# kzhai/PyLDA

Hardware: AMD Instinct MI355X
Metric: documents/sec per VB iteration (higher is better)
Workload: dtype f64

## Files before the change

include/pylda_hip.h:

```cpp
#ifndef PYLDA_HIP_H
#define PYLDA_HIP_H

#include <stdint.h>

#ifdef __cplusplus
extern "C" {
#endif

typedef struct pylda_ctx pylda_ctx;
typedef struct pylda_corpus pylda_corpus;

typedef enum pylda_status {
    PYLDA_OK = 0,
    PYLDA_ERR_INVALID = -1,
    PYLDA_ERR_HIP = -2,
    PYLDA_ERR_OOM = -3,
    PYLDA_ERR_STATE = -4
} pylda_status;

#define PYLDA_ABI_VERSION 10
int pylda_abi_version(void);

const char* pylda_version(void);

// ... 77 lines not shown
int pylda_work_counters(pylda_ctx* ctx, double* inner_iterations, double* inner_iteration_terms);
int pylda_executed_work(pylda_ctx* ctx, double* tile_entries, double* handed_over);
int pylda_stop_sum_counters(pylda_ctx* ctx, double* skipped, double* formed);
int pylda_clock_counters(pylda_ctx* ctx, double* shader_ticks, double* wall_ticks, double* wall_hz);

int pylda_corpus_plan(pylda_corpus* corpus, int32_t capacity, int32_t* variant, int32_t* geometry,
                      int64_t* documents, int64_t* terms, double* kernel_ms);

int64_t pylda_corpus_layout(pylda_corpus* corpus, const char* name);

int pylda_set_option(pylda_ctx* ctx, const char* name, int64_t value);

int pylda_test_special(pylda_ctx* ctx, int64_t n, const double* x, double* digamma_out,
                       double* lgamma_out);

int pylda_parse_corpus(const char* text, int64_t text_bytes, int doc_separator, const char* vocab,
                       int64_t vocab_bytes, int lowercase, int64_t* n_docs, int64_t* nnz,
                       int64_t* doc_ptr, int32_t* term_id, int32_t* term_ct, int64_t* dropped_docs);

int pylda_test_alpha_update(pylda_ctx* ctx, const double* alpha_k, const double* alpha_ss_k, double number_of_documents,
                            int hyper_parameter_iteration, double hyper_parameter_decay_factor,
                            int hyper_parameter_maximum_decay, double hyper_parameter_converge_threshold,
                            double* alpha_out_k);

int pylda_hybrid_estep(pylda_ctx* ctx, pylda_corpus* corpus, int number_of_samples, int burn_in_samples, uint64_t seed,
                       uint64_t stream, int64_t first_document, int heldout);
int pylda_hybrid_scale_sstats(pylda_ctx* ctx, double divisor);

int pylda_test_philox(pylda_ctx* ctx, int64_t n, const uint32_t* counter_key, uint32_t* out);

int pylda_gibbs_init(pylda_ctx* ctx, pylda_corpus* corpus, uint64_t seed, int64_t first_document);
int pylda_gibbs_sweep(pylda_ctx* ctx, pylda_corpus* corpus, const double* alpha_k, const double* beta_v, double beta_sum,
                      int64_t blocks, uint64_t seed, uint64_t stream, int64_t first_document);
int pylda_gibbs_log_posterior(pylda_ctx* ctx, pylda_corpus* corpus, const double* alpha_k, const double* beta_v, double* out);
int pylda_gibbs_get_counts(pylda_ctx* ctx, pylda_corpus* corpus, int32_t* n_kv, int32_t* n_k, int32_t* topics);
int pylda_gibbs_set_state(pylda_ctx* ctx, pylda_corpus* corpus, const int32_t* n_kv, const int32_t* n_k, const int32_t* topics);

int pylda_gibbs_round_tokens(pylda_ctx* ctx, pylda_corpus* corpus, int64_t blocks, int64_t first_document, int64_t* tokens);
int pylda_gibbs_exchange_prepare(pylda_ctx* ctx, pylda_corpus* corpus, int64_t blocks, int64_t first_document, int world, int rank,
                                 const int64_t* capacity, void** send, void** recv);
int pylda_gibbs_round_sample(pylda_ctx* ctx, pylda_corpus* corpus, const double* alpha_k, const double* beta_v, double beta_sum,
                             int64_t blocks, int64_t round, uint64_t seed, uint64_t stream, int64_t first_document);
int pylda_gibbs_round_apply(pylda_ctx* ctx, pylda_corpus* corpus, int64_t round);
int pylda_gibbs_table_device(pylda_ctx* ctx, pylda_corpus* corpus, void** table, int64_t* table_elements, void** n_k);
int pylda_gibbs_log_posterior_parts(pylda_ctx* ctx, pylda_corpus* corpus, const double* alpha_k, const double* beta_v, double* out);

// ... 59 lines not shown
```

pylda_amd/_capi.py:

```python
import collections
import ctypes
import os
import threading

import numpy as np

ABI_VERSION = 10
_LIB_PATH = os.path.join(os.path.dirname(os.path.abspath(__file__)), "lib", "libpylda_hip.so")
_lib = None

_c_double_p = ctypes.POINTER(ctypes.c_double)
_c_int32_p = ctypes.POINTER(ctypes.c_int32)
_c_int64_p = ctypes.POINTER(ctypes.c_int64)
_vp = ctypes.c_void_p

SIGNATURES = {
    "pylda_version": (ctypes.c_char_p, []),
    "pylda_abi_version": (ctypes.c_int, []),
    "pylda_device_count": (ctypes.c_int, [ctypes.POINTER(ctypes.c_int)]),
    "pylda_create": (ctypes.c_int, [ctypes.c_int, ctypes.c_int, ctypes.c_int, ctypes.POINTER(_vp)]),
    "pylda_destroy": (None, [_vp]),
    "pylda_last_error": (ctypes.c_char_p, [_vp]),
    "pylda_set_stream": (ctypes.c_int, [_vp, _vp]),
    "pylda_use_own_stream": (ctypes.c_int, [_vp]),
# ... 38 lines not shown
    "pylda_host_free": (ctypes.c_int, [_vp]),
    "pylda_model_checkpoint": (ctypes.c_int, [_vp, ctypes.c_int]),
    "pylda_mark_time": (ctypes.c_int, [_vp, ctypes.c_int]),
    "pylda_elapsed_ms": (ctypes.c_int, [_vp, ctypes.c_int, ctypes.c_int, _c_double_p]),
    "pylda_work_counters": (ctypes.c_int, [_vp, _c_double_p, _c_double_p]),
    "pylda_executed_work": (ctypes.c_int, [_vp, _c_double_p, _c_double_p]),
    "pylda_stop_sum_counters": (ctypes.c_int, [_vp, _c_double_p, _c_double_p]),
    "pylda_clock_counters": (ctypes.c_int, [_vp, _c_double_p, _c_double_p, _c_double_p]),
    "pylda_set_profiling": (ctypes.c_int, [_vp, ctypes.c_int]),
    "pylda_kernel_time": (ctypes.c_int, [_vp, _c_double_p, _c_double_p, _c_int64_p]),
    "pylda_corpus_layout": (ctypes.c_int64, [_vp, ctypes.c_char_p]),
    "pylda_corpus_plan": (ctypes.c_int, [_vp, ctypes.c_int32, _c_int32_p, _c_int32_p, _c_int64_p, _c_int64_p,
                                         _c_double_p]),
    "pylda_set_option": (ctypes.c_int, [_vp, ctypes.c_char_p, ctypes.c_int64]),
    "pylda_parse_corpus": (ctypes.c_int, [ctypes.c_char_p, ctypes.c_int64, ctypes.c_int, ctypes.c_char_p,
                                          ctypes.c_int64, ctypes.c_int, _c_int64_p, _c_int64_p, _c_int64_p,
                                          _c_int32_p, _c_int32_p, _c_int64_p]),
    "pylda_test_alpha_update": (ctypes.c_int, [_vp, _c_double_p, _c_double_p, ctypes.c_double, ctypes.c_int, ctypes.c_double,
                                               ctypes.c_int, ctypes.c_double, _c_double_p]),
    "pylda_test_expdigamma": (ctypes.c_int, [_vp, ctypes.c_int64, _c_double_p, ctypes.c_double, _c_double_p]),
    "pylda_test_special_forms": (ctypes.c_int, [_vp, ctypes.c_int64, _c_double_p, ctypes.c_double, ctypes.c_int, _c_double_p]),
    "pylda_test_tables": (ctypes.c_int, [_vp, _c_double_p, _c_double_p, _c_double_p, _c_double_p, _c_double_p, _c_double_p,
                                         _c_double_p, ctypes.POINTER(ctypes.c_int)]),
    "pylda_test_statistics": (ctypes.c_int, [_vp, _vp, _c_double_p, _c_double_p, _c_int32_p, ctypes.POINTER(ctypes.c_uint16),
                                             _c_double_p, _c_double_p]),
    "pylda_test_special": (ctypes.c_int, [_vp, ctypes.c_int64, _c_double_p, _c_double_p, _c_double_p]),
    "pylda_test_gibbs_posterior_terms": (ctypes.c_int, [_vp, _vp, _c_double_p, _c_double_p, _c_double_p, _c_double_p, _c_double_p]),
    "pylda_hybrid_estep": (ctypes.c_int, [_vp, _vp, ctypes.c_int, ctypes.c_int, ctypes.c_uint64, ctypes.c_uint64,
                                          ctypes.c_int64, ctypes.c_int]),
    "pylda_hybrid_scale_sstats": (ctypes.c_int, [_vp, ctypes.c_double]),
    "pylda_test_philox": (ctypes.c_int, [_vp, ctypes.c_int64, ctypes.POINTER(ctypes.c_uint32),
                                         ctypes.POINTER(ctypes.c_uint32)]),
    "pylda_gibbs_init": (ctypes.c_int, [_vp, _vp, ctypes.c_uint64, ctypes.c_int64]),
    "pylda_gibbs_sweep": (ctypes.c_int, [_vp, _vp, _c_double_p, _c_double_p, ctypes.c_double, ctypes.c_int64, ctypes.c_uint64,
                                         ctypes.c_uint64, ctypes.c_int64]),
    "pylda_gibbs_log_posterior": (ctypes.c_int, [_vp, _vp, _c_double_p, _c_double_p, _c_double_p]),
    "pylda_gibbs_get_counts": (ctypes.c_int, [_vp, _vp, _c_int32_p, _c_int32_p, _c_int32_p]),
    "pylda_gibbs_set_state": (ctypes.c_int, [_vp, _vp, _c_int32_p, _c_int32_p, _c_int32_p]),
    "pylda_gibbs_round_tokens": (ctypes.c_int, [_vp, _vp, ctypes.c_int64, ctypes.c_int64, _c_int64_p]),
    "pylda_gibbs_exchange_prepare": (ctypes.c_int, [_vp, _vp, ctypes.c_int64, ctypes.c_int64, ctypes.c_int, ctypes.c_int, _c_int64_p,
                                                    ctypes.POINTER(_vp), ctypes.POINTER(_vp)]),
    "pylda_gibbs_round_sample": (ctypes.c_int, [_vp, _vp, _c_double_p, _c_double_p, ctypes.c_double, ctypes.c_int64, ctypes.c_int64,
                                                ctypes.c_uint64, ctypes.c_uint64, ctypes.c_int64]),
    "pylda_gibbs_round_apply": (ctypes.c_int, [_vp, _vp, ctypes.c_int64]),
    "pylda_gibbs_table_device": (ctypes.c_int, [_vp, _vp, ctypes.POINTER(_vp), _c_int64_p, ctypes.POINTER(_vp)]),
    "pylda_gibbs_log_posterior_parts": (ctypes.c_int, [_vp, _vp, _c_double_p, _c_double_p, _c_double_p]),
# ... 624 lines not shown

    def allreduce_doubles(self, values):
        values = np.ascontiguousarray(values, dtype=np.float64).copy()
        self._check(self._lib.pylda_allreduce_doubles(self._h, _dp(values), values.size))
        return values

    def set_profiling(self, enabled):
        self._check(self._lib.pylda_set_profiling(self._h, 1 if enabled else 0))

    def kernel_time(self):
        ms, ss, calls = ctypes.c_double(0), ctypes.c_double(0), ctypes.c_int64(0)
        self._check(self._lib.pylda_kernel_time(self._h, ctypes.byref(ms), ctypes.byref(ss), ctypes.byref(calls)))
        return ms.value, ss.value, calls.value

    def test_alpha_update(self, alpha, alpha_ss, number_of_documents, iterations=100, decay_factor=0.9, maximum_decay=10,
                          threshold=1e-6):
        alpha, alpha_ss = _f64(alpha, (self.K,), "alpha"), _f64(alpha_ss, (self.K,), "alpha_ss")
        out = np.empty(self.K, dtype=np.float64)
        self._check(self._lib.pylda_test_alpha_update(self._h, _dp(alpha), _dp(alpha_ss), float(number_of_documents),
                                                      int(iterations), float(decay_factor), int(maximum_decay),
                                                      float(threshold), _dp(out)))
        return out

    def test_expdigamma(self, x, c):
        x = _f64(x)
        out = np.empty_like(x)
        self._check(self._lib.pylda_test_expdigamma(self._h, x.size, _dp(x), float(c), _dp(out)))
        return out

    def test_special_forms(self, x, form, c=0.0):
        x = _f64(x)
        out = np.empty_like(x)
        self._check(self._lib.pylda_test_special_forms(self._h, x.size, _dp(x), float(c), int(form), _dp(out)))
        return out

    def test_special(self, x):
        x = _f64(x)
        dg, lg = np.empty_like(x), np.empty_like(x)
        self._check(self._lib.pylda_test_special(self._h, x.size, _dp(x), _dp(dg), _dp(lg)))
        return dg, lg

    def test_tables(self, alpha_sgn=False, tables=True, only=None):
        ldk = int(self._lib.pylda_table_stride(self._h))
        out = {}
        if tables:
            out = {"psi_rowsum": (self.K,), "elog": (self.V, ldk), "expElog": (self.V, ldk),
# ... 117 lines not shown
```

pylda_amd/csrc/context.hip:

```cpp
#include "host_internal.h"
#include "transpose_kernel.h"
#include "special_device.h"

namespace pylda_host {

std::string g_create_error;

int fail(pylda_ctx* ctx, int code, const char* fmt, ...)
{
    char buf[512];
    va_list ap;
    va_start(ap, fmt);
    vsnprintf(buf, sizeof buf, fmt, ap);
    va_end(ap);
    if (ctx) ctx->err = buf; else g_create_error = buf;
    return code;
}

static hipEvent_t take_event(pylda_ctx* ctx)
{
    if (!ctx->event_pool.empty()) {
        hipEvent_t e = ctx->event_pool.back();
        ctx->event_pool.pop_back();
        return e;
// ... 138 lines not shown
    for (int i = 0; i < pylda_ctx::kAux; ++i) {
        CREATE_TRY(hip_ok(hipStreamCreateWithFlags(&ctx->aux_stream[i], hipStreamNonBlocking), "hipStreamCreate"));
        CREATE_TRY(hip_ok(hipEventCreateWithFlags(&ctx->join_event[i], hipEventDisableTiming), "hipEventCreate"));
    }
    CREATE_TRY(hip_ok(hipEventCreateWithFlags(&ctx->fork_event, hipEventDisableTiming), "hipEventCreate"));
    const size_t kv = (size_t)K * V, wk = (size_t)V * ctx->ldk;
    CREATE_TRY(dev_alloc(ctx, &ctx->d_eta, kv));
    CREATE_TRY(dev_alloc(ctx, &ctx->d_elog, wk));
    CREATE_TRY(dev_alloc(ctx, &ctx->d_expElog, wk));
    CREATE_TRY(dev_alloc(ctx, &ctx->d_expElog_elog, wk));
    CREATE_TRY(dev_alloc(ctx, &ctx->d_sstats, wk));
    CREATE_TRY(dev_alloc(ctx, &ctx->d_kv_scratch, kv));
    CREATE_TRY(dev_alloc(ctx, &ctx->d_shift, (size_t)V));
    CREATE_TRY(dev_alloc(ctx, &ctx->d_beta, (size_t)V));
    CREATE_TRY(dev_alloc(ctx, &ctx->d_psi_rowsum, (size_t)K));
    CREATE_TRY(dev_alloc(ctx, &ctx->d_topic_lse, (size_t)K));
    CREATE_TRY(dev_alloc(ctx, &ctx->d_alpha, (size_t)K));
    CREATE_TRY(dev_alloc(ctx, &ctx->d_alpha_sgn, (size_t)K));
    CREATE_TRY(dev_alloc(ctx, &ctx->d_alpha_wsum, (size_t)1));
    CREATE_TRY(dev_alloc(ctx, &ctx->d_small, (size_t)(4 * K + 16)));
    CREATE_TRY(dev_alloc(ctx, &ctx->d_partial, (size_t)1024 * K));
    CREATE_TRY(dev_alloc(ctx, &ctx->d_outer, (size_t)(3 * K + 8)));
    CREATE_TRY(dev_alloc(ctx, &ctx->d_newton_work, (size_t)4 * K));
    CREATE_TRY(dev_alloc(ctx, &ctx->d_work, (size_t)8));
    CREATE_TRY(hip_ok(hipMemsetAsync(ctx->d_work, 0, 8 * sizeof(double), ctx->stream), "hipMemsetAsync"));
    CREATE_TRY(hip_ok(hipHostMalloc(reinterpret_cast<void**>(&ctx->h_pin), (size_t)(5 * K + 8) * sizeof(double), hipHostMallocDefault),
                      "hipHostMalloc"));
    for (int i = 0; i < 2; ++i)
        CREATE_TRY(hip_ok(hipEventCreateWithFlags(&ctx->alpha_event[i], hipEventDisableTiming), "hipEventCreate"));
    CREATE_TRY(hip_ok(hipMemsetAsync(ctx->d_sstats, 0, wk * sizeof(double), ctx->stream),
                      "hipMemsetAsync"));
#undef CREATE_TRY
    *out = ctx;
    return PYLDA_OK;
}

void pylda_destroy(pylda_ctx* ctx)
{
    if (!ctx) return;
    (void)hipSetDevice(ctx->device);
    if (ctx->own_stream) (void)hipStreamSynchronize(ctx->own_stream);
    if (ctx->comm) pylda::comm_destroy(ctx->comm);
    dev_free(ctx->d_comm_small);
    dev_free(ctx->d_foldin_table); dev_free(ctx->d_foldin_alpha); dev_free(ctx->d_completion_rowsum);
    dev_free(ctx->d_similarity_base);
    dev_free(ctx->d_ltr_z); dev_free(ctx->d_ltr_p);
    drain_events(ctx);
// ... 79 lines not shown
        ctx->wide_postings = value != 0;
    } else if (!strcmp(name, "lds_pad")) {
        ctx->lds_pad = (int)value;
    } else if (!strcmp(name, "quad")) {
        ctx->quad = value != 0;
        ctx->plan_epoch += 1;
    } else if (!strcmp(name, "quad_stream")) {
        ctx->quad_stream = value != 0;
        ctx->plan_epoch += 1;
    } else if (!strcmp(name, "quad_packed")) {
        ctx->quad_packed = value != 0;
    } else if (!strcmp(name, "prepare_path")) {
        if (value < 0 || value > 2 || (value == 1 && ctx->K > 64))
            return fail(ctx, PYLDA_ERR_INVALID, "prepare_path=%lld at K=%d: 0 (by size), 1 (one kernel, K <= 64) or 2 (two passes)",
                        (long long)value, ctx->K);
        ctx->prepare_path = (int)value;
    } else if (!strcmp(name, "quilt12")) {
        ctx->quilt12 = value != 0;
        ctx->plan_epoch += 1;
    } else if (!strcmp(name, "doc_values")) {
        ctx->doc_values = value != 0;
    } else if (!strcmp(name, "gather_live")) {
        ctx->gather_live = value != 0;
    } else if (!strcmp(name, "compact")) {
        ctx->compact = value != 0;
    } else if (!strcmp(name, "compact_pair")) {
        ctx->compact_pair = value < 0 ? -1 : value != 0;
    } else if (!strcmp(name, "compact_stream")) {
        ctx->compact_stream = value != 0;
    } else if (!strcmp(name, "compact_phase")) {
        ctx->compact_phase = value != 0;
    } else if (!strcmp(name, "compact_cap")) {
        if (value < 0 || value > kLiveStride) return fail(ctx, PYLDA_ERR_INVALID, "compact_cap=%lld: 0 .. %d", (long long)value, kLiveStride);
        ctx->compact_cap = (int)value;
    } else if (!strcmp(name, "compact_guard_fail")) {
        ctx->compact_guard_fail = value != 0;
    } else if (!strcmp(name, "compact_underflow_doc")) {
        ctx->compact_underflow_doc = value;
    } else if (!strcmp(name, "coherence_chunk_docs")) {
        if (value < 0 || value % 64) return fail(ctx, PYLDA_ERR_INVALID, "coherence_chunk_docs=%lld: a multiple of 64, or 0", (long long)value);
        ctx->coherence_chunk_docs = value;
    } else if (!strcmp(name, "similarity_doc_slices")) {
        if (value < 0 || value > 1024) return fail(ctx, PYLDA_ERR_INVALID, "similarity_doc_slices=%lld: 1 .. 1024, or 0", (long long)value);
        ctx->similarity_doc_slices = (int)value;
    } else if (!strcmp(name, "topic_distance_segment_groups")) {
        if (value < 0 || value > 65535)
// ... 393 lines not shown
```

pylda_amd/csrc/doc_terms.h:

```cpp
#pragma once
#include "estep_common.h"
#include "special_device.h"

namespace pylda {

__global__ __launch_bounds__(256) void doc_terms_kernel(EstepParams p, int64_t count)
{
    const int lane = threadIdx.x & (kWave - 1);
    const int64_t slot = (int64_t)blockIdx.x * (256 / kWave) + threadIdx.x / kWave;
    if (slot >= count) return;
    const int64_t doc = p.order ? p.order[slot] : slot;
    if (p.status[doc] != 3) return;
    const int K = p.K;
    const double* gamma = p.gamma + (size_t)doc * K;
    const double* t = p.tfinal + (size_t)doc * p.ldk;
    double lgam = 0.0, gsum = 0.0, term2 = 0.0, term3 = 0.0;
    const int listed = p.live_stats ? p.live_n[doc] : -1;
    if (listed >= 0) {
        if (lane < listed) {
            char* list = live_list_of(p.live_list, doc);
            const int k = *live_idx_at(list, lane);
            const double g = gamma[k], a = p.alpha[k], mass = g - a;
            lgam = lgamma_pos(g) - lgamma_pos(a);
            gsum = mass;
// ... 7 lines not shown
            if (mass != 0.0) term2 = fma(log(t[k]), mass, term2);
        }
    }
    const int64_t lo = p.doc_ptr[doc], hi = p.doc_ptr[doc + 1];
    for (int64_t n = lo + lane; n < hi; n += kWave) {
        const double c = (double)p.term_ct[n];
        term3 = fma(c, log(c) - log(p.rfinal[n]), term3);
    }
    lgam = wave_sum(lgam);
    gsum = wave_sum(gsum);
    if (listed >= 0) {
        lgam += p.alpha_lgamma_sum;
        gsum += p.alpha_sum;
    }
    term2 = wave_sum(term2);
    term3 = wave_sum(term3);
    if (lane == 0) {
        p.doc_ll[doc] = p.alpha_term + lgam - lgamma_pos(gsum) - (term2 - term3);
        p.doc_words_ll[doc] = 0.0;
        p.status[doc] = 0;
    }
}

__global__ __launch_bounds__(1024) void work_count_kernel(const int32_t* __restrict__ iters, const int64_t* __restrict__ doc_ptr,
                                                          int64_t D, double* __restrict__ work, const int32_t* __restrict__ handoff_it,
                                                          const int32_t* __restrict__ col_iters, int K)
{
    __shared__ double scratch[16];
    const long long tick0 = clock64(), wall0 = wall_clock64();
    double a = 0.0, b = 0.0, e = 0.0, h = 0.0, sc = 0.0, fs = 0.0;
    for (int64_t d = threadIdx.x; d < D; d += 1024) {
        const double it = (double)iters[d], n = (double)(doc_ptr[d + 1] - doc_ptr[d]);
        a += it;
        b += it * n;
        const int at = handoff_it ? handoff_it[d] : -1;
        if (at >= 0) {
            const int cols = col_iters[d] & ((1 << kColItersShift) - 1), skipped = col_iters[d] >> kColItersShift;
            e += n * ((double)K * at + (double)cols);
            h += 1.0;
            sc += (double)skipped;
            fs += it - (double)at - (double)skipped;
        } else {
            e += n * (double)K * it;
        }
    }
    a = block_sum<1024>(a, scratch);
    b = block_sum<1024>(b, scratch);
    e = block_sum<1024>(e, scratch);
    h = block_sum<1024>(h, scratch);
    sc = block_sum<1024>(sc, scratch);
    fs = block_sum<1024>(fs, scratch);
    if (threadIdx.x == 0) {
        work[0] += a;
        work[1] += b;
        work[2] += e;
        work[3] += h;
        work[4] += (double)(clock64() - tick0);
        work[5] += (double)(wall_clock64() - wall0);
        work[6] += sc;
        work[7] += fs;
    }
}

}
```

pylda_amd/csrc/estep_api.hip:

```cpp
#include "host_internal.h"
#include "estep_logspace.h"
#include "doc_terms.h"
#include "prepare_kernels.h"

namespace pylda_host {

int prepare_path_of(const pylda_ctx* ctx)
{
    if (ctx->prepare_path) return ctx->prepare_path;
    return ctx->K <= 64 && (int64_t)ctx->K * ctx->V <= (1 << 21) ? 1 : 2;
}

int enqueue_prepare(pylda_ctx* ctx, bool heldout)
{
    const int K = ctx->K, V = ctx->V;
    hipLaunchKernelGGL(eta_rowsum_psi_kernel, dim3(K), dim3(256), 0, ctx->stream, ctx->d_eta, K, V,
                       ctx->d_psi_rowsum);
    if (prepare_path_of(ctx) == 1) {
        hipLaunchKernelGGL(elog_rows_small_kernel, dim3((V + 3) / 4), dim3(256), 0, ctx->stream, ctx->d_eta, ctx->d_psi_rowsum,
                           K, V, ctx->ldk, ctx->d_elog, ctx->d_expElog, ctx->d_expElog_elog, ctx->d_shift);
    } else {
        hipLaunchKernelGGL(elog_transpose_kernel, dim3((V + 31) / 32, (K + 31) / 32), dim3(256), 0,
                           ctx->stream, ctx->d_eta, ctx->d_psi_rowsum, K, V, ctx->ldk, ctx->d_elog);
        hipLaunchKernelGGL(row_shift_exp_kernel, dim3((V + 3) / 4), dim3(256), 0, ctx->stream,
// ... 489 lines not shown
    if (!(tol >= 0.0) && !(tol < 0.0)) return fail(ctx, PYLDA_ERR_INVALID, "estep: threshold is NaN");
    if (!ctx->have_eta || !ctx->have_alpha)
        return fail(ctx, PYLDA_ERR_STATE, "estep: set_eta and set_alpha must be called first");
    HIP_TRY(ctx, hipSetDevice(ctx->device));
    heldout = heldout ? 1 : 0;
    int rc = enqueue_prepare(ctx, heldout != 0);
    if (rc != PYLDA_OK) return rc;
    if ((rc = estep_plan(ctx, c, tol, heldout != 0)) != PYLDA_OK) return rc;
    EstepParams p = estep_params(ctx, c, max_iter, tol, heldout);
    if ((rc = reset_handoff(ctx, c, p)) != PYLDA_OK) return rc;
    if (ctx->profiling && ctx->class_ms.size() != c->plan.size()) ctx->class_ms.assign(c->plan.size(), 0.0);
    const int doc_bracket = open_bracket(ctx, -1, ctx->stream);
    if (ctx->force_logspace) {
        HIP_TRY(ctx, hipMemsetD32Async(reinterpret_cast<hipDeviceptr_t>(c->d_status), 1, (size_t)c->D, ctx->stream));
    } else {
        if ((rc = enqueue_dense_classes(ctx, c, p)) != PYLDA_OK) return rc;
        if ((rc = enqueue_live_phase(ctx, c, p)) != PYLDA_OK) return rc;
    }
    const bool terms_forked = enqueue_doc_terms(ctx, c, p);
    close_bracket(ctx, doc_bracket, ctx->stream);
    if (ctx->profiling) ctx->estep_calls += 1;
    if (!heldout && (rc = enqueue_statistics(ctx, c, terms_forked)) != PYLDA_OK) return rc;
    if ((rc = enqueue_logspace_net(ctx, c, p)) != PYLDA_OK) return rc;
    if (ctx->profiling && c->D > 0)
        hipLaunchKernelGGL(work_count_kernel, dim3(1), dim3(1024), 0, ctx->stream, c->d_iters, c->d_doc_ptr, c->D, ctx->d_work,
                           c->compact_ready ? c->d_handoff_it : nullptr, c->d_col_iters, ctx->K);
    return finish_estep(ctx, c, heldout, !heldout, p.want_doc_ll != 0);
}

int pylda_estep_results(pylda_ctx* ctx, pylda_corpus* c, double* document_log_likelihood,
                        double* words_log_likelihood, int64_t* logspace_documents)
{
    if (!ctx) return PYLDA_ERR_INVALID;
    if (!c || c->ctx != ctx) return fail(ctx, PYLDA_ERR_INVALID, "estep_results: bad corpus");
    if (!c->estep_done) return fail(ctx, PYLDA_ERR_STATE, "estep_results: no E-step has run on this corpus");
    HIP_TRY(ctx, hipSetDevice(ctx->device));
    double* sc = ctx->h_pin + (size_t)5 * ctx->K + 4;
    int32_t* nflag_pin = reinterpret_cast<int32_t*>(sc + 3);
    HIP_TRY(ctx, hipMemcpyAsync(sc, c->d_scalars, 4 * sizeof(double), hipMemcpyDeviceToHost, ctx->stream));
    HIP_TRY(ctx, hipStreamSynchronize(ctx->stream));
    const int32_t nflag = *nflag_pin;
    if (!c->last_doc_values) sc[0] -= sc[2];
    if (document_log_likelihood) *document_log_likelihood = sc[0];
    if (words_log_likelihood) *words_log_likelihood = sc[1];
    if (logspace_documents) *logspace_documents = nflag;
    return PYLDA_OK;
}

int pylda_get_gamma(pylda_ctx* ctx, pylda_corpus* c, double* gamma_dk)
// ... 149 lines not shown
```

pylda_amd/csrc/estep_limits.h:

```cpp
#pragma once
#if defined(__HIPCC__)
#include <hip/hip_runtime.h>
#elif !defined(__host__)
#define __host__
#define __device__
#endif
#include <stddef.h>
#include <stdint.h>

namespace pylda {

struct GenericLds {
    size_t tile, t, lt, gam, r, lognrm, cts, ids, red, scratch, total;
};

__host__ __device__ inline GenericLds generic_lds_layout(int K, int n_cap, int tile_stride,
                                                          int nthreads, bool tile_global)
{
    auto a16 = [](size_t x) { return (x + 15) & ~(size_t)15; };
    GenericLds L;
    size_t off = 0;
    L.tile = off;   off = a16(off + (tile_global ? 0 : (size_t)n_cap * tile_stride * 8));
    L.t = off;      off = a16(off + (size_t)K * 8);
    L.lt = off;     off = a16(off + (size_t)K * 8);
// ... 3 lines not shown
    L.cts = off;    off = a16(off + (size_t)n_cap * 8);
    L.ids = off;    off = a16(off + (size_t)n_cap * 4);
    int kl = 1;
    while (kl < K && kl < nthreads) kl <<= 1;
    int groups = nthreads / kl;
    L.red = off;    off = a16(off + (size_t)groups * K * 8);
    L.scratch = off; off = a16(off + (size_t)(nthreads / 64) * 8);
    L.total = off;
    return L;
}

__host__ __device__ inline size_t logspace_lds_bytes(int K)
{
    return (size_t)(6 * K + 4) * 8 + 64;
}
constexpr size_t kLdsMargin = 3072;
constexpr int kLogspaceListDocs = 256;
__host__ __device__ inline size_t logspace_list_offset(int K) { return (logspace_lds_bytes(K) + 15) & ~(size_t)15; }
__host__ __device__ inline size_t logspace_launch_lds_bytes(int K)
{
    return logspace_list_offset(K) + (size_t)(kLogspaceListDocs + 1) * sizeof(int32_t);
}

#ifndef PYLDA_QF_SLOTS
#define PYLDA_QF_SLOTS 128
#endif
constexpr int kQfMaxSlots = PYLDA_QF_SLOTS;

constexpr int kQgMaxWords = 1024;

__host__ __device__ constexpr int quad_slot_term(int s, int gg, int wpr) { return s * 16 + (s < wpr ? gg : 15 - gg); }
__host__ __device__ constexpr int quad_wpr_of(int rn) { return rn % 10000 / 100 + rn % 100; }
__host__ __device__ constexpr int quad_wpg_of(int rn) { return quad_wpr_of(rn) + rn / 1000000; }
__host__ __device__ constexpr bool quad_packs_slots(int tl) { return tl == 32; }
__host__ __device__ constexpr int quad_tl_of(int rn) { return rn % 1000000 / 10000; }
__host__ __device__ constexpr int quad_ids_stride(int wpg) { return (wpg + 3) & ~3; }
__host__ __device__ constexpr int64_t quad_ids_at(int64_t slot, int gg, int stride) { return (slot * 16 + gg) * stride; }
#ifndef PYLDA_QUAD_PROLOGUE_AT_ONCE
#define PYLDA_QUAD_PROLOGUE_AT_ONCE 1
#endif
#ifndef PYLDA_QUAD_EARLY_HANDOFF
#define PYLDA_QUAD_EARLY_HANDOFF 1
#endif
__host__ __device__ constexpr bool quad_prologue_at_once(int tl) { return PYLDA_QUAD_PROLOGUE_AT_ONCE && tl == 32; }
__host__ __device__ constexpr bool quad_early_handoff(int tl) { return PYLDA_QUAD_EARLY_HANDOFF && tl == 32; }
#ifndef PYLDA_LIVE_STOP_SHORTCUT
// ... 27 lines not shown
```

pylda_amd/csrc/host_internal.h:

```cpp
#pragma once
#include "../../include/pylda_hip.h"

#include <hip/hip_runtime.h>

#include <algorithm>
#include <chrono>
#include <cmath>
#include <cstdarg>
#include <cstdio>
#include <cstdlib>
#include <cstring>
#include <new>
#include <numeric>
#include <string>
#include <thread>
#include <vector>

#include "comm.h"
#include "estep_common.h"
#include "estep_limits.h"
#include "host_plan.h"
#include "postings.h"

using namespace pylda;
// ... 70 lines not shown
    int force_logspace = 0;
    int force_variant = -1;
    int quilt12 = 0;
    int gather_rows = 2;
    int gather_blocks = -1;
    int sweep_xcd = 1;
    int sweep_sub = 4;
    int sweep_spin = 4000;
    int gather_sweep = 1;
    int gather_round_mb = 0;
    int launch_order = 1;
    int terms_overlap = 1;
    int slab_uber = 1;
    int wide_postings = 0;
    int lds_pad = 0;
    int quad = 1;
    int quad_stream = 1;
    int prepare_path = 0;
    int quad_packed = 1;
    int quilt_odd = 1;
    int doc_values = 1;
    int compact = 1;
    int gather_live = 1;
    int compact_phase = 1;
    int compact_stream = 1;
    int compact_pair = -1;
    int compact_cap = 0;
    int compact_guard_fail = 0;
    int64_t compact_underflow_doc = -1;
    int64_t coherence_chunk_docs = 0;
    int similarity_doc_slices = 0;
    double* d_similarity_base = nullptr;
    int64_t similarity_D = 0;
    int topic_distance_segment_groups = 0;
    int plan_epoch = 0;
    bool exact_stop = false;

    struct Bracket { hipEvent_t a, b; int slot; };
    bool profiling = false;
    std::vector<Bracket> pending_events;
    std::vector<hipEvent_t> event_pool;
    double doc_kernel_ms = 0.0, sstats_kernel_ms = 0.0;
    std::vector<double> class_ms;
    int64_t estep_calls = 0;

    std::string err;
// ... 207 lines not shown
```

pylda_amd/csrc/mstep_api.hip:

```cpp
#include "host_internal.h"
#include "mstep_kernels.h"

extern "C" {

namespace {
struct OnlineBlend { double rho, omr, scale; };

static int enqueue_mstep(pylda_ctx* ctx, pylda_corpus* c, const double* beta_v, bool want_alpha_ss, const char* who,
                         const OnlineBlend* blend = nullptr)
{
    if (!beta_v) return fail(ctx, PYLDA_ERR_INVALID, "%s: beta is NULL", who);
    if (!ctx->have_eta || !ctx->have_sstats)
        return fail(ctx, PYLDA_ERR_STATE, "%s: needs eta and the sufficient statistics of a training E-step", who);
    if (want_alpha_ss && (!c || c->ctx != ctx || !c->estep_done))
        return fail(ctx, PYLDA_ERR_STATE, "%s: alpha statistics need the corpus of the last E-step", who);
    HIP_TRY(ctx, hipSetDevice(ctx->device));
    const int K = ctx->K, V = ctx->V;
    if (ctx->h_beta.size() != (size_t)V || memcmp(ctx->h_beta.data(), beta_v, (size_t)V * sizeof(double)) != 0) {
        double bsum = 0.0, blg = 0.0;
        for (int v = 0; v < V; ++v) {
            if (!(beta_v[v] > 0.0)) return fail(ctx, PYLDA_ERR_INVALID, "%s: beta[%d]=%g", who, v, beta_v[v]);
            bsum += beta_v[v];
            blg += std::lgamma(beta_v[v]);
        }
        ctx->h_beta.clear();
        HIP_TRY(ctx, hipMemcpyAsync(ctx->d_beta, beta_v, (size_t)V * sizeof(double), hipMemcpyHostToDevice, ctx->stream));
        HIP_TRY(ctx, hipStreamSynchronize(ctx->stream));
        ctx->h_beta.assign(beta_v, beta_v + V);
        ctx->beta_sum = bsum;
        ctx->beta_lgamma_sum = blg;
    }
    double* d_per_topic = ctx->d_small;
    double* d_alpha_ss = ctx->d_small + K;
    hipLaunchKernelGGL(mstep_topic_ll_kernel, dim3(K, kTopicChunks), dim3(256), 0, ctx->stream, ctx->d_eta, K, V,
                       ctx->d_partial);
    hipLaunchKernelGGL(mstep_topic_ll_finish_kernel, dim3((K + 255) / 256), dim3(256), 0, ctx->stream, ctx->d_partial, K,
                       d_per_topic);
    if (blend)
        hipLaunchKernelGGL(mstep_online_eta_kernel, dim3((K + 31) / 32, (V + 31) / 32), dim3(256), 0, ctx->stream,
                           ctx->d_sstats, ctx->d_beta, K, V, ctx->ldk, blend->rho, blend->omr, blend->scale, ctx->d_eta);
    else
        hipLaunchKernelGGL(mstep_update_eta_kernel, dim3((K + 31) / 32, (V + 31) / 32), dim3(256), 0, ctx->stream,
                           ctx->d_sstats, ctx->d_beta, K, V, ctx->ldk, ctx->d_eta);
    if (want_alpha_ss) {
        const int nblocks = (int)std::min<int64_t>(1024, std::max<int64_t>(1, (c->D + 3) / 4));
        hipLaunchKernelGGL(mstep_alpha_ss_kernel, dim3(nblocks), dim3(256), (size_t)4 * K * sizeof(double),
                           ctx->stream, c->d_gamma, c->D, K, ctx->d_partial);
        hipLaunchKernelGGL(column_sum_kernel, dim3((K + 63) / 64), dim3(256), 0, ctx->stream, ctx->d_partial,
                           nblocks, K, d_alpha_ss);
    }
    HIP_TRY(ctx, hipGetLastError());
    return PYLDA_OK;
}

static double topic_ll_from(const pylda_ctx* ctx, const double* per_topic)
{
    double ll = ctx->K * (std::lgamma(ctx->beta_sum) - ctx->beta_lgamma_sum);
    for (int k = 0; k < ctx->K; ++k) ll += per_topic[k];
    return ll;
}
}

int pylda_mstep(pylda_ctx* ctx, pylda_corpus* c, const double* beta_v, double* topic_log_likelihood,
                double* alpha_ss_k)
{
    if (!ctx) return PYLDA_ERR_INVALID;
    const int rc = enqueue_mstep(ctx, c, beta_v, alpha_ss_k != nullptr, "mstep");
    if (rc != PYLDA_OK) return rc;
    const int K = ctx->K;
    std::vector<double> per_topic((size_t)K);
    HIP_TRY(ctx, hipMemcpyAsync(per_topic.data(), ctx->d_small, (size_t)K * sizeof(double), hipMemcpyDeviceToHost, ctx->stream));
    if (alpha_ss_k)
// ... 138 lines not shown
    const int K = ctx->K;
    double* d = nullptr;
    int rc = dev_alloc(ctx, &d, (size_t)3 * K + 1);
    if (rc != PYLDA_OK) return rc;
    NewtonParams np;
    np.iterations = hyper_parameter_iteration;
    np.maximum_decay = hyper_parameter_maximum_decay;
    np.threshold = hyper_parameter_converge_threshold;
    for (int i = 0; i <= 16; ++i) np.decay_power[i] = std::pow(hyper_parameter_decay_factor, (double)i);
    hipError_t e = hipMemcpy(d, alpha_k, (size_t)K * sizeof(double), hipMemcpyHostToDevice);
    if (e == hipSuccess) e = hipMemcpy(d + K, alpha_ss_k, (size_t)K * sizeof(double), hipMemcpyHostToDevice);
    if (e == hipSuccess) e = hipMemcpy(d + 2 * (size_t)K, &number_of_documents, sizeof(double), hipMemcpyHostToDevice);
    if (e == hipSuccess) {
        hipLaunchKernelGGL(alpha_newton_kernel, dim3(1), dim3(1024), 0, ctx->stream, d, d + K, d + 2 * (size_t)K, K, np,
                           ctx->d_newton_work, d + 2 * (size_t)K + 1);
        e = hipStreamSynchronize(ctx->stream);
    }
    if (e == hipSuccess) e = hipMemcpy(alpha_out_k, d, (size_t)K * sizeof(double), hipMemcpyDeviceToHost);
    dev_free(d);
    if (e != hipSuccess) return fail(ctx, PYLDA_ERR_HIP, "test_alpha_update: %s", hipGetErrorString(e));
    return PYLDA_OK;
}

}
```

pylda_amd/csrc/mstep_kernels.h:

```cpp
#pragma once
#include "estep_common.h"
#include "special_device.h"
#include "estep_limits.h"

namespace pylda {

constexpr int kTopicChunks = 8;
__global__ __launch_bounds__(256) void mstep_topic_ll_kernel(const double* __restrict__ eta, int K,
                                                             int V, double* __restrict__ part)
{
    __shared__ double scratch[4];
    const int k = blockIdx.x, chunk = blockIdx.y;
    const int per = (V + kTopicChunks - 1) / kTopicChunks;
    const int v0 = chunk * per, v1 = min(V, v0 + per);
    const double* row = eta + (size_t)k * V;
    double lg = 0.0, s = 0.0;
    for (int v = v0 + threadIdx.x; v < v1; v += 256) {
        const double e = row[v];
        lg += lgamma_pos(e);
        s += e;
    }
    lg = block_sum<256>(lg, scratch);
    s = block_sum<256>(s, scratch);
    if (threadIdx.x == 0) {
// ... 75 lines not shown
    for (int k = lane; k < K; k += kWave) acc[wave * K + k] = 0.0;
    const int64_t stride = (int64_t)gridDim.x * 4;
    for (int64_t d = (int64_t)blockIdx.x * 4 + wave; d < D; d += 2 * stride) {
        const double* g0 = gamma + (size_t)d * K;
        const bool two = d + stride < D;
        const double* g1 = two ? gamma + (size_t)(d + stride) * K : g0;
        double s0 = 0.0, s1 = 0.0;
        for (int k = lane; k < K; k += kWave) {
            s0 += g0[k];
            s1 += g1[k];
        }
        s0 = wave_sum(s0);
        s1 = wave_sum(s1);
        const double ps0 = digamma(s0), ps1 = digamma(s1);
        for (int k = lane; k < K; k += kWave) {
            double a = acc[wave * K + k] + (digamma(g0[k]) - ps0);
            if (two) a += digamma(g1[k]) - ps1;
            acc[wave * K + k] = a;
        }
    }
    __syncthreads();
    for (int k = threadIdx.x; k < K; k += 256)
        partial[(size_t)blockIdx.x * K + k] = acc[k] + acc[K + k] + acc[2 * K + k] + acc[3 * K + k];
}

__global__ __launch_bounds__(256) void column_sum_kernel(const double* __restrict__ partial,
                                                         int nblocks, int K,
                                                         double* __restrict__ out)
{
    __shared__ double part[4][64];
    const int kk = threadIdx.x & 63, grp = threadIdx.x >> 6;
    const int k = blockIdx.x * 64 + kk;
    double s = 0.0;
    if (k < K)
        for (int b = grp; b < nblocks; b += 4) s += partial[(size_t)b * K + k];
    part[grp][kk] = s;
    __syncthreads();
    if (grp == 0 && k < K) out[k] = (part[0][kk] + part[1][kk]) + (part[2][kk] + part[3][kk]);
}

__global__ __launch_bounds__(256) void outer_pack_kernel(const double* __restrict__ scalars, const int32_t* __restrict__ flag_count,
                                                         int doc_values, double n_docs, const double* __restrict__ alpha_ss,
                                                         const double* __restrict__ per_topic, const double* __restrict__ alpha,
                                                         int K, double* __restrict__ out)
{
    if (threadIdx.x == 0) {
// ... 80 lines not shown
```

Measured before the change: 5.077 million.

## Skip digamma for gamma entries equal to alpha in alpha sufficient statistics

Adds an alpha-statistics kernel that detects, per document, which gamma entries differ bitwise from alpha. Only those moved entries are compacted into a per-wave list and passed through digamma; the rest reuse a precomputed digamma(alpha) table held in LDS. This targets the per-element digamma cost in the M-step, in exchange for ballot and compaction overhead and a larger LDS footprint. It also spreads the profiling work-count reduction across many blocks with a second reduce kernel, and adds a test entry point and an option to turn the new path off.

```diff
diff --git a/include/pylda_hip.h b/include/pylda_hip.h
--- a/include/pylda_hip.h
+++ b/include/pylda_hip.h
@@ -123,6 +123,8 @@
                             int hyper_parameter_iteration, double hyper_parameter_decay_factor,
                             int hyper_parameter_maximum_decay, double hyper_parameter_converge_threshold,
                             double* alpha_out_k);
+
+int pylda_test_alpha_statistics(pylda_ctx* ctx, const double* gamma_dk, int64_t D, double* out_k);
 
 int pylda_hybrid_estep(pylda_ctx* ctx, pylda_corpus* corpus, int number_of_samples, int burn_in_samples, uint64_t seed,
                        uint64_t stream, int64_t first_document, int heldout);
diff --git a/pylda_amd/_capi.py b/pylda_amd/_capi.py
--- a/pylda_amd/_capi.py
+++ b/pylda_amd/_capi.py
@@ -84,6 +84,7 @@
     "pylda_test_special_forms": (ctypes.c_int, [_vp, ctypes.c_int64, _c_double_p, ctypes.c_double, ctypes.c_int, _c_double_p]),
     "pylda_test_tables": (ctypes.c_int, [_vp, _c_double_p, _c_double_p, _c_double_p, _c_double_p, _c_double_p, _c_double_p,
                                          _c_double_p, ctypes.POINTER(ctypes.c_int)]),
+    "pylda_test_alpha_statistics": (ctypes.c_int, [_vp, _c_double_p, ctypes.c_int64, _c_double_p]),
     "pylda_test_statistics": (ctypes.c_int, [_vp, _vp, _c_double_p, _c_double_p, _c_int32_p, ctypes.POINTER(ctypes.c_uint16),
                                              _c_double_p, _c_double_p]),
     "pylda_test_special": (ctypes.c_int, [_vp, ctypes.c_int64, _c_double_p, _c_double_p, _c_double_p]),
@@ -754,6 +755,14 @@
                                                       float(threshold), _dp(out)))
         return out
 
+    def test_alpha_statistics(self, gamma):
+        gamma = np.ascontiguousarray(gamma, dtype=np.float64)
+        if gamma.ndim != 2 or gamma.shape[1] != self.K:
+            raise ValueError("gamma has shape %s, expected (D, %d)" % (gamma.shape, self.K))
+        out = np.empty(self.K, dtype=np.float64)
+        self._check(self._lib.pylda_test_alpha_statistics(self._h, _dp(gamma), gamma.shape[0], _dp(out)))
+        return out
+
     def test_expdigamma(self, x, c):
         x = _f64(x)
         out = np.empty_like(x)
diff --git a/pylda_amd/csrc/context.hip b/pylda_amd/csrc/context.hip
--- a/pylda_amd/csrc/context.hip
+++ b/pylda_amd/csrc/context.hip
@@ -184,7 +184,7 @@
     CREATE_TRY(dev_alloc(ctx, &ctx->d_partial, (size_t)1024 * K));
     CREATE_TRY(dev_alloc(ctx, &ctx->d_outer, (size_t)(3 * K + 8)));
     CREATE_TRY(dev_alloc(ctx, &ctx->d_newton_work, (size_t)4 * K));
-    CREATE_TRY(dev_alloc(ctx, &ctx->d_work, (size_t)8));
+    CREATE_TRY(dev_alloc(ctx, &ctx->d_work, (size_t)8 + 8 * kWorkCountBlocks));
     CREATE_TRY(hip_ok(hipMemsetAsync(ctx->d_work, 0, 8 * sizeof(double), ctx->stream), "hipMemsetAsync"));
     CREATE_TRY(hip_ok(hipHostMalloc(reinterpret_cast<void**>(&ctx->h_pin), (size_t)(5 * K + 8) * sizeof(double), hipHostMallocDefault),
                       "hipHostMalloc"));
@@ -310,6 +310,8 @@
         ctx->doc_values = value != 0;
     } else if (!strcmp(name, "gather_live")) {
         ctx->gather_live = value != 0;
+    } else if (!strcmp(name, "alpha_ss_moved")) {
+        ctx->alpha_ss_moved = value != 0;
     } else if (!strcmp(name, "compact")) {
         ctx->compact = value != 0;
     } else if (!strcmp(name, "compact_pair")) {
diff --git a/pylda_amd/csrc/doc_terms.h b/pylda_amd/csrc/doc_terms.h
--- a/pylda_amd/csrc/doc_terms.h
+++ b/pylda_amd/csrc/doc_terms.h
@@ -53,14 +53,14 @@
     }
 }
 
-__global__ __launch_bounds__(1024) void work_count_kernel(const int32_t* __restrict__ iters, const int64_t* __restrict__ doc_ptr,
-                                                          int64_t D, double* __restrict__ work, const int32_t* __restrict__ handoff_it,
-                                                          const int32_t* __restrict__ col_iters, int K)
+__global__ __launch_bounds__(1024) void work_count_partial_kernel(const int32_t* __restrict__ iters, const int64_t* __restrict__ doc_ptr,
+                                                                  int64_t D, double* __restrict__ part, const int32_t* __restrict__ handoff_it,
+                                                                  const int32_t* __restrict__ col_iters, int K)
 {
     __shared__ double scratch[16];
     const long long tick0 = clock64(), wall0 = wall_clock64();
     double a = 0.0, b = 0.0, e = 0.0, h = 0.0, sc = 0.0, fs = 0.0;
-    for (int64_t d = threadIdx.x; d < D; d += 1024) {
+    for (int64_t d = (int64_t)blockIdx.x * 1024 + threadIdx.x; d < D; d += (int64_t)gridDim.x * 1024) {
         const double it = (double)iters[d], n = (double)(doc_ptr[d + 1] - doc_ptr[d]);
         a += it;
         b += it * n;
@@ -82,14 +82,33 @@
     sc = block_sum<1024>(sc, scratch);
     fs = block_sum<1024>(fs, scratch);
     if (threadIdx.x == 0) {
-        work[0] += a;
-        work[1] += b;
-        work[2] += e;
-        work[3] += h;
-        work[4] += (double)(clock64() - tick0);
-        work[5] += (double)(wall_clock64() - wall0);
-        work[6] += sc;
-        work[7] += fs;
+        double* row = part + (size_t)blockIdx.x * 8;
+        row[0] = a;
+        row[1] = b;
+        row[2] = e;
+        row[3] = h;
+        row[4] = (double)(clock64() - tick0);
+        row[5] = (double)(wall_clock64() - wall0);
+        row[6] = sc;
+        row[7] = fs;
+    }
+}
+
+__global__ __launch_bounds__(512) void work_count_kernel(const double* __restrict__ part, int rows, double* __restrict__ work)
+{
+    __shared__ double group[64][8];
+    const long long tick0 = clock64(), wall0 = wall_clock64();
+    const int j = threadIdx.x & 7, grp = threadIdx.x >> 3;
+    double s = 0.0;
+    for (int b = grp; b < rows; b += 64) s += part[(size_t)b * 8 + j];
+    group[grp][j] = s;
+    __syncthreads();
+    if (threadIdx.x < 8) {
+        double total = 0.0;
+        for (int g = 0; g < 64; ++g) total += group[g][j];
+        if (j == 4) total += (double)(clock64() - tick0);
+        if (j == 5) total += (double)(wall_clock64() - wall0);
+        work[j] += total;
     }
 }
 
diff --git a/pylda_amd/csrc/estep_api.hip b/pylda_amd/csrc/estep_api.hip
--- a/pylda_amd/csrc/estep_api.hip
+++ b/pylda_amd/csrc/estep_api.hip
@@ -535,9 +535,12 @@
     if (ctx->profiling) ctx->estep_calls += 1;
     if (!heldout && (rc = enqueue_statistics(ctx, c, terms_forked)) != PYLDA_OK) return rc;
     if ((rc = enqueue_logspace_net(ctx, c, p)) != PYLDA_OK) return rc;
-    if (ctx->profiling && c->D > 0)
-        hipLaunchKernelGGL(work_count_kernel, dim3(1), dim3(1024), 0, ctx->stream, c->d_iters, c->d_doc_ptr, c->D, ctx->d_work,
-                           c->compact_ready ? c->d_handoff_it : nullptr, c->d_col_iters, ctx->K);
+    if (ctx->profiling && c->D > 0) {
+        const int rows = (int)std::min<int64_t>(kWorkCountBlocks, (c->D + 1023) / 1024);
+        hipLaunchKernelGGL(work_count_partial_kernel, dim3(rows), dim3(1024), 0, ctx->stream, c->d_iters, c->d_doc_ptr, c->D,
+                           ctx->d_work + 8, c->compact_ready ? c->d_handoff_it : nullptr, c->d_col_iters, ctx->K);
+        hipLaunchKernelGGL(work_count_kernel, dim3(1), dim3(512), 0, ctx->stream, ctx->d_work + 8, rows, ctx->d_work);
+    }
     return finish_estep(ctx, c, heldout, !heldout, p.want_doc_ll != 0);
 }
 
diff --git a/pylda_amd/csrc/estep_limits.h b/pylda_amd/csrc/estep_limits.h
--- a/pylda_amd/csrc/estep_limits.h
+++ b/pylda_amd/csrc/estep_limits.h
@@ -49,6 +49,8 @@
     return logspace_list_offset(K) + (size_t)(kLogspaceListDocs + 1) * sizeof(int32_t);
 }
 
+constexpr int kWorkCountBlocks = 1024;
+
 #ifndef PYLDA_QF_SLOTS
 #define PYLDA_QF_SLOTS 128
 #endif
diff --git a/pylda_amd/csrc/host_internal.h b/pylda_amd/csrc/host_internal.h
--- a/pylda_amd/csrc/host_internal.h
+++ b/pylda_amd/csrc/host_internal.h
@@ -116,6 +116,7 @@
     int doc_values = 1;
     int compact = 1;
     int gather_live = 1;
+    int alpha_ss_moved = 1;
     int compact_phase = 1;
     int compact_stream = 1;
     int compact_pair = -1;
diff --git a/pylda_amd/csrc/mstep_api.hip b/pylda_amd/csrc/mstep_api.hip
--- a/pylda_amd/csrc/mstep_api.hip
+++ b/pylda_amd/csrc/mstep_api.hip
@@ -5,6 +5,22 @@
 
 namespace {
 struct OnlineBlend { double rho, omr, scale; };
+
+static int enqueue_alpha_statistics(pylda_ctx* ctx, const double* d_gamma, int64_t D, double* out_k)
+{
+    const int K = ctx->K;
+    const int nblocks = (int)std::min<int64_t>(1024, std::max<int64_t>(1, (D + 3) / 4));
+    if (ctx->alpha_ss_moved && alpha_ss_moved_lds(K) + kLdsMargin <= ctx->lds_limit)
+        HIP_TRY(ctx, launch_kernel(mstep_alpha_ss_moved_kernel, dim3(nblocks), dim3(256), alpha_ss_moved_lds(K), ctx->stream,
+                                   d_gamma, (const double*)ctx->d_alpha, D, K, ctx->d_partial));
+    else
+        hipLaunchKernelGGL(mstep_alpha_ss_kernel, dim3(nblocks), dim3(256), (size_t)4 * K * sizeof(double),
+                           ctx->stream, d_gamma, D, K, ctx->d_partial);
+    hipLaunchKernelGGL(column_sum_kernel, dim3((K + 63) / 64), dim3(256), 0, ctx->stream, ctx->d_partial,
+                       nblocks, K, out_k);
+    HIP_TRY(ctx, hipGetLastError());
+    return PYLDA_OK;
+}
 
 static int enqueue_mstep(pylda_ctx* ctx, pylda_corpus* c, const double* beta_v, bool want_alpha_ss, const char* who,
                          const OnlineBlend* blend = nullptr)
@@ -43,11 +59,8 @@
         hipLaunchKernelGGL(mstep_update_eta_kernel, dim3((K + 31) / 32, (V + 31) / 32), dim3(256), 0, ctx->stream,
                            ctx->d_sstats, ctx->d_beta, K, V, ctx->ldk, ctx->d_eta);
     if (want_alpha_ss) {
-        const int nblocks = (int)std::min<int64_t>(1024, std::max<int64_t>(1, (c->D + 3) / 4));
-        hipLaunchKernelGGL(mstep_alpha_ss_kernel, dim3(nblocks), dim3(256), (size_t)4 * K * sizeof(double),
-                           ctx->stream, c->d_gamma, c->D, K, ctx->d_partial);
-        hipLaunchKernelGGL(column_sum_kernel, dim3((K + 63) / 64), dim3(256), 0, ctx->stream, ctx->d_partial,
-                           nblocks, K, d_alpha_ss);
+        const int rc = enqueue_alpha_statistics(ctx, c->d_gamma, c->D, d_alpha_ss);
+        if (rc != PYLDA_OK) return rc;
     }
     HIP_TRY(ctx, hipGetLastError());
     return PYLDA_OK;
@@ -232,4 +245,30 @@
     return PYLDA_OK;
 }
 
-}
+int pylda_test_alpha_statistics(pylda_ctx* ctx, const double* gamma_dk, int64_t D, double* out_k)
+{
+    if (!ctx) return PYLDA_ERR_INVALID;
+    if (D < 0 || (D > 0 && !gamma_dk) || !out_k) return fail(ctx, PYLDA_ERR_INVALID, "test_alpha_statistics: bad argument");
+    if (!ctx->have_alpha) return fail(ctx, PYLDA_ERR_STATE, "test_alpha_statistics: set_alpha must be called first");
+    HIP_TRY(ctx, hipSetDevice(ctx->device));
+    const int K = ctx->K;
+    double* d_gamma = nullptr;
+    int rc = dev_alloc(ctx, &d_gamma, std::max<size_t>(1, (size_t)D * K));
+    if (rc != PYLDA_OK) return rc;
+    hipError_t e = hipSuccess;
+    if (D > 0) e = hipMemcpyAsync(d_gamma, gamma_dk, (size_t)D * K * sizeof(double), hipMemcpyHostToDevice, ctx->stream);
+    if (e == hipSuccess) e = hipMemsetAsync(ctx->d_partial, 0xff, (size_t)1024 * K * sizeof(double), ctx->stream);
+    if (e == hipSuccess) e = hipMemsetAsync(ctx->d_small + K, 0xff, (size_t)K * sizeof(double), ctx->stream);
+    if (e == hipSuccess) {
+        rc = enqueue_alpha_statistics(ctx, d_gamma, D, ctx->d_small + K);
+        if (rc == PYLDA_OK) e = hipMemcpyAsync(out_k, ctx->d_small + K, (size_t)K * sizeof(double), hipMemcpyDeviceToHost, ctx->stream);
+    }
+    const hipError_t waited = hipStreamSynchronize(ctx->stream);
+    dev_free(d_gamma);
+    if (rc != PYLDA_OK) return rc;
+    if (e == hipSuccess) e = waited;
+    if (e != hipSuccess) return fail(ctx, PYLDA_ERR_HIP, "test_alpha_statistics: %s", hipGetErrorString(e));
+    return PYLDA_OK;
+}
+
+}
diff --git a/pylda_amd/csrc/mstep_kernels.h b/pylda_amd/csrc/mstep_kernels.h
--- a/pylda_amd/csrc/mstep_kernels.h
+++ b/pylda_amd/csrc/mstep_kernels.h
@@ -121,6 +121,131 @@
     __syncthreads();
     for (int k = threadIdx.x; k < K; k += 256)
         partial[(size_t)blockIdx.x * K + k] = acc[k] + acc[K + k] + acc[2 * K + k] + acc[3 * K + k];
+}
+
+__host__ __device__ inline size_t alpha_ss_moved_lds(int K)
+{
+    const size_t stripes = (size_t)(K + kWave - 1) / kWave;
+    return ((size_t)6 * K + 8 * (kWave + stripes)) * sizeof(double) + (size_t)8 * kWave * sizeof(int32_t);
+}
+
+__device__ __forceinline__ double alpha_ss_list_terms(const double* list_g, const int32_t* list_k, int from, int n, double ps,
+                                                      bool ps_rides, double* acc, int lane)
+{
+    wave_lds_exchange();
+    const double psi = digamma(lane < n ? list_g[lane] : 1.0);
+    const double first = __shfl(psi, 0, kWave);
+    if (ps_rides) ps = first;
+    if (lane >= from && lane < n) {
+        const int k = list_k[lane];
+        acc[k] = acc[k] + (psi - ps);
+    }
+    wave_lds_exchange();
+    return first;
+}
+
+__device__ __forceinline__ void alpha_ss_document(const double* __restrict__ g, double s, int n, double* list_g, int32_t* list_k,
+                                                  const unsigned long long* moved, double* acc,
+                                                  const double* psi_alpha, int K, int stripes, int lane)
+{
+    const unsigned long long below = (1ull << lane) - 1;
+    double ps;
+    if (n <= kWave) {
+        if (lane == 0) list_g[0] = s;
+        ps = alpha_ss_list_terms(list_g, list_k, 1, n, 0.0, true, acc, lane);
+    } else {
+        ps = digamma(s);
+        int cnt = 0;
+        for (int j = 0; j < stripes; ++j) {
+            const unsigned long long mv = moved[j];
+            const unsigned long long m = (unsigned long long)(unsigned)__builtin_amdgcn_readfirstlane((int)(mv >> 32)) << 32 |
+                                         (unsigned)__builtin_amdgcn_readfirstlane((int)mv);
+            const int c = __popcll(m);
+            if (c == 0) continue;
+            if (cnt + c > kWave) {
+                alpha_ss_list_terms(list_g, list_k, 0, cnt, ps, false, acc, lane);
+                cnt = 0;
+            }
+            if ((m >> lane) & 1) {
+                const int k = j * kWave + lane, at = cnt + __popcll(m & below);
+                list_g[at] = g[k];
+                list_k[at] = k;
+            }
+            cnt += c;
+        }
+        alpha_ss_list_terms(list_g, list_k, 0, cnt, ps, false, acc, lane);
+    }
+    for (int j = 0, k = lane; k < K; ++j, k += kWave)
+        if (!((moved[j] >> lane) & 1)) acc[k] = acc[k] + (psi_alpha[k] - ps);
+}
+
+__global__ __launch_bounds__(256) void mstep_alpha_ss_moved_kernel(const double* __restrict__ gamma,
+                                                                   const double* __restrict__ alpha, int64_t D, int K,
+                                                                   double* __restrict__ partial)
+{
+    extern __shared__ __attribute__((aligned(16))) char smem[];
+    const int lane = threadIdx.x & (kWave - 1), wave = threadIdx.x / kWave;
+    const int stripes = (K + kWave - 1) / kWave;
+    double* acc_all = reinterpret_cast<double*>(smem);
+    double* alpha_s = acc_all + (size_t)4 * K;
+    double* psi_alpha = alpha_s + K;
+    double* list_g = psi_alpha + K + (size_t)wave * 2 * kWave;
+    unsigned long long* moved = reinterpret_cast<unsigned long long*>(psi_alpha + K + 8 * kWave) + (size_t)wave * 2 * stripes;
+    int32_t* list_k = reinterpret_cast<int32_t*>(psi_alpha + K + 8 * kWave + (size_t)8 * stripes) + wave * 2 * kWave;
+    double* acc = acc_all + (size_t)wave * K;
+    for (int k = threadIdx.x; k < K; k += 256) {
+        const double a = alpha[k];
+        alpha_s[k] = a;
+        psi_alpha[k] = digamma(a);
+    }
+    for (int k = lane; k < K; k += kWave) acc[k] = 0.0;
+    __syncthreads();
+    const unsigned long long below = (1ull << lane) - 1;
+    const int64_t stride = (int64_t)gridDim.x * 4;
+    for (int64_t d = (int64_t)blockIdx.x * 4 + wave; d < D; d += 2 * stride) {
+        const double* g0 = gamma + (size_t)d * K;
+        const bool two = d + stride < D;
+        const double* g1 = two ? gamma + (size_t)(d + stride) * K : g0;
+        double s0 = 0.0, s1 = 0.0;
+        int n0 = 1, n1 = 1;
+        for (int j = 0; j < stripes; ++j) {
+            const int k = j * kWave + lane;
+            const bool in = k < K;
+            const double x0 = in ? g0[k] : 0.0, x1 = in ? g1[k] : 0.0;
+            const long long a = in ? __double_as_longlong(alpha_s[k]) : 0;
+            if (in) {
+                s0 += x0;
+                s1 += x1;
+            }
+            const unsigned long long m0 = __ballot(in && __double_as_longlong(x0) != a);
+            const unsigned long long m1 = __ballot(in && __double_as_longlong(x1) != a);
+            if (lane == 0) {
+                moved[j] = m0;
+                moved[stripes + j] = m1;
+            }
+            const int c0 = __popcll(m0), c1 = __popcll(m1);
+            if (n0 + c0 <= kWave && ((m0 >> lane) & 1)) {
+                const int at = n0 + __popcll(m0 & below);
+                list_g[at] = x0;
+                list_k[at] = k;
+            }
+            if (n1 + c1 <= kWave && ((m1 >> lane) & 1)) {
+                const int at = n1 + __popcll(m1 & below);
+                list_g[kWave + at] = x1;
+                list_k[kWave + at] = k;
+            }
+            n0 += c0;
+            n1 += c1;
+        }
+        s0 = wave_sum(s0);
+        s1 = wave_sum(s1);
+        wave_lds_exchange();
+        alpha_ss_document(g0, s0, n0, list_g, list_k, moved, acc, psi_alpha, K, stripes, lane);
+        if (two) alpha_ss_document(g1, s1, n1, list_g + kWave, list_k + kWave, moved + stripes, acc, psi_alpha, K, stripes, lane);
+    }
+    __syncthreads();
+    for (int k = threadIdx.x; k < K; k += 256)
+        partial[(size_t)blockIdx.x * K + k] = acc_all[k] + acc_all[K + k] + acc_all[2 * K + k] + acc_all[3 * K + k];
 }
 
 __global__ __launch_bounds__(256) void column_sum_kernel(const double* __restrict__ partial,
```

Result: faster. 5.145 million, median of 6 (+1.3%).
